# rednote-hilab/dots.ocr

Hardware: AMD Instinct MI355X
Metric: pages/sec, dots.ocr 1.7B bf16, A4@200dpi page batch (preprocess + ViT + prefill + 1024-token greedy decode + detokenise) (higher is better)
Workload: dtype bf16; 1 GPU; a4: 8 pages/GPU of 1654x2339 px -> 19824 patches, 5200 prompt tokens/page, max_new_tokens=1024, EOS disabled; pages_per_gpu=8, parallelism=dp1, decode_rows_in_flight=64

## Files before the change

### dots_ocr_amd/csrc/elementwise.hip

```cpp
#include "common.h"
#include "kernels.h"

namespace {

constexpr int MAX_CHUNKS = 8;

template <bool LAYERNORM, int NCH>
__global__ __launch_bounds__(256) void norm_kernel(const bf16_t* __restrict__ x, const bf16_t* __restrict__ w,
                                                   const bf16_t* __restrict__ b, bf16_t* __restrict__ y,
                                                   int64_t rows, int dim, float eps) {
    const int l = threadIdx.x & 63;
    const int64_t row = (int64_t)blockIdx.x * 4 + (threadIdx.x >> 6);
    if (row >= rows) return;
    const bf16_t* xr = x + row * dim;
    constexpr int NC = NCH > 0 ? NCH : MAX_CHUNKS;
    u32x4 v[NC];
    float s = 0.f, s2 = 0.f;
    if constexpr (NCH > 0) {
#pragma unroll
        for (int c = 0; c < NC; ++c) v[c] = *reinterpret_cast<const u32x4*>(xr + c * 512 + l * 8);
    }
#pragma unroll
    for (int c = 0; c < NC; ++c) {
        const int off = c * 512 + l * 8;
// ... 134 lines not shown
            const int item = it * 256 + tid;
            const int tok = item >> 4, c = item & 15;
            u32x4 v = {0, 0, 0, 0};
            if (tok < tl.n) v = *reinterpret_cast<const u32x4*>(qkv + (size_t)(tl.tok0 + tok) * ld + (Hq + Hkv + h) * 128 + c * 8);
            const int p = (tok & ~15) | (tok & 3) | (((tok >> 3) & 1) << 2) | (((tok >> 2) & 1) << 3);
            *reinterpret_cast<u32x4*>(&lds[p * 136 + c * 8]) = v;
        }
        __syncthreads();
#pragma unroll
        for (int it = 0; it < 4; ++it) {
            const int item = it * 256 + tid;
            const int d = item >> 3, pc = item & 7;
            u32x4 o;
#pragma unroll
            for (int e = 0; e < 4; ++e) {
                uint32_t a = lds[(pc * 8 + 2 * e) * 136 + d], b = lds[(pc * 8 + 2 * e + 1) * 136 + d];
                o[e] = a | (b << 16);
            }
            *reinterpret_cast<u32x4*>(vt + ((size_t)h * 128 + d) * Tpad + tl.pad0 + pc * 8) = o;
        }
    }
}

__global__ __launch_bounds__(256) void embed_gather_kernel(const int32_t* __restrict__ src, const bf16_t* __restrict__ embed,
                                                           const bf16_t* __restrict__ vision, bf16_t* __restrict__ x,
                                                           int64_t T, int dim) {
    const int l = threadIdx.x & 63;
    const int64_t t = (int64_t)blockIdx.x * 4 + (threadIdx.x >> 6);
    if (t >= T) return;
    const int sidx = src[t];
    const bf16_t* s = sidx >= 0 ? embed + (size_t)sidx * dim : vision + (size_t)(-sidx - 1) * dim;
    for (int off = l * 8; off < dim; off += 512)
        *reinterpret_cast<u32x4*>(x + t * dim + off) = *reinterpret_cast<const u32x4*>(s + off);
}

__global__ __launch_bounds__(256) void gather_rows_kernel(const bf16_t* __restrict__ x, const int32_t* __restrict__ rows,
                                                          const int32_t* __restrict__ dst, bf16_t* __restrict__ y, int n, int dim) {
    const int l = threadIdx.x & 63;
    const int r = blockIdx.x * 4 + (threadIdx.x >> 6);
    if (r >= n) return;
    const bf16_t* s = x + (size_t)rows[r] * dim;
    bf16_t* d = y + (size_t)(dst ? dst[r] : r) * dim;
    for (int off = l * 8; off < dim; off += 512) *reinterpret_cast<u32x4*>(d + off) = *reinterpret_cast<const u32x4*>(s + off);
}

}
// ... 23 lines not shown
hipError_t launch_patch_prep(hipStream_t s, const float* x, bf16_t* y, int64_t rows, int in_dim, int out_dim) {
    if (rows <= 0) return hipSuccess;
    if (in_dim % 4 != 0 || out_dim % 4 != 0 || out_dim < in_dim) return hipErrorInvalidValue;
    const int64_t n = rows * (out_dim / 4);
    hipLaunchKernelGGL(patch_prep_kernel, dim3((unsigned)((n + 255) / 256)), dim3(256), 0, s, x, y, rows, in_dim, out_dim);
    return hipGetLastError();
}

hipError_t launch_rope_table(hipStream_t s, const int32_t* pos, const float* inv_freq, float2* cs, int64_t T, int two_d) {
    if (T <= 0) return hipSuccess;
    hipLaunchKernelGGL(rope_table_kernel, dim3((unsigned)((T * 64 + 255) / 256)), dim3(256), 0, s, pos, inv_freq, cs, T, two_d);
    return hipGetLastError();
}

hipError_t launch_qkv_rope_split(hipStream_t s, const bf16_t* qkv, const float2* cs, const Tile64* tiles, int n_tiles,
                                 bf16_t* q, bf16_t* k, bf16_t* vt, int64_t T, int64_t Tpad, int Hq, int Hkv, bool v_only) {
    if (n_tiles <= 0) return hipSuccess;
    const int n_groups = (Hq + Hkv + ROPE_HPB - 1) / ROPE_HPB;
    if (v_only) hipLaunchKernelGGL(qkv_rope_split_kernel, dim3(n_tiles, Hkv), dim3(256), 0, s, qkv, cs, tiles, q, k, vt, T, Tpad, Hq, Hkv, n_groups);
    else hipLaunchKernelGGL(qkv_rope_split_kernel, dim3(n_tiles, n_groups + Hkv), dim3(256), 0, s, qkv, cs, tiles, q, k, vt, T, Tpad, Hq, Hkv, 0);
    return hipGetLastError();
}

hipError_t launch_embed_gather(hipStream_t s, const int32_t* src, const bf16_t* embed, const bf16_t* vision, bf16_t* x,
                               int64_t T, int dim) {
    if (T <= 0) return hipSuccess;
    hipLaunchKernelGGL(embed_gather_kernel, dim3((unsigned)((T + 3) / 4)), dim3(256), 0, s, src, embed, vision, x, T, dim);
    return hipGetLastError();
}

hipError_t launch_gather_rows(hipStream_t s, const bf16_t* x, const int32_t* rows, const int32_t* dst, bf16_t* y, int n, int dim) {
    if (n <= 0) return hipSuccess;
    hipLaunchKernelGGL(gather_rows_kernel, dim3((n + 3) / 4), dim3(256), 0, s, x, rows, dst, y, n, dim);
    return hipGetLastError();
}
```

### dots_ocr_amd/csrc/engine.hip

```cpp
#include <hip/hip_runtime.h>
#include <hip/hip_fp16.h>

#include <algorithm>
#include <cmath>
#include <cstdarg>
#include <cstddef>
#include <cstdio>
#include <cstdlib>
#include <cstring>
#include <string>
#include <unordered_map>
#include <vector>

#include "common.h"
#include "decode_layout.h"
#include "dots_ocr_hip.h"
#include "kernels.h"

namespace {

thread_local std::string g_create_error;

struct Tensor {
    bf16_t* p = nullptr;
// ... 86 lines not shown
    hipEvent_t ev_vis_ready = nullptr, ev_xs = nullptr;
    bf16_t* vis_pref = nullptr;
    int64_t vis_pref_rows = 0;
    bool pref_pending = false;
    bool pref_deferred = false;
    const float* pref_pix = nullptr;
    int64_t pref_patches = 0;
    std::vector<int64_t> pref_grid;
    hipStream_t vs = nullptr;
    hipStream_t s_vit_full = nullptr;
    hipEvent_t ev_tw0 = nullptr, ev_tw_sw = nullptr, ev_dec_end = nullptr;
    int tail_fixed = 0;
    int tail_now = 0;
    int tail_head_blocks = 0;
    uint64_t tw_seq = 0, dec_end_seq = 0, dec_end_at_tw = 0;
    std::vector<LLayer> ll;
    float *v_inv_freq = nullptr, *lm_inv_freq = nullptr;

    int64_t P = 0, Ppad = 0;
    bf16_t *v_xa = nullptr, *v_x = nullptr, *v_xn = nullptr, *v_qkv = nullptr, *v_q = nullptr, *v_k = nullptr, *v_vt = nullptr,
           *v_att = nullptr, *v_act = nullptr, *v_mh = nullptr, *vis = nullptr;
    float* v_pix = nullptr;
    float2* v_cs = nullptr;
    int32_t* v_pos = nullptr;
    Tile64* v_tiles = nullptr;
    QBlock* v_qblocks = nullptr;
    int64_t vis_rows = 0;
    std::vector<int32_t> h_pos;
    std::vector<Tile64> h_tiles;
    std::vector<QBlock> h_qblocks;

    int64_t TP = 0, TPpad = 0;
    bf16_t *p_x = nullptr, *p_xn = nullptr, *p_qkv = nullptr, *p_q = nullptr, *p_k = nullptr, *p_vt = nullptr, *p_att = nullptr, *p_act = nullptr;
    float2* p_cs = nullptr;
    int32_t *p_pos = nullptr, *p_src = nullptr, *p_last = nullptr;
    Tile64* p_tiles = nullptr;
    QBlock* p_qblocks = nullptr;
    std::vector<int32_t> hp_pos, hp_src, hp_last, hp_table;
    std::vector<Tile64> hp_tiles;
    std::vector<QBlock> hp_qblocks;

    int max_pages = 0;
    int n_pool_pages = 0;
    int kv_capped = 0;
    std::vector<int32_t> free_pages;
    std::vector<std::vector<int32_t>> slot_pages;
    bf16_t* pool = nullptr;
// ... 156 lines not shown
    return DOTS_OK;
}

int dense_on(DotsEngine* e, hipStream_t st, uint8_t* aq, float* as, const bf16_t* A, const bf16_t* W, const uint8_t* W8, const float* wscale,
             const bf16_t* bias, const bf16_t* R, void* C, int64_t M, int N, int K, int ldc, int epi) {
    if (!W8) {
        CK(launch_gemm(st, A, W, bias, R, C, M, N, K, K, ldc, epi, wscale));
        return DOTS_OK;
    }
    CK(launch_quant_act_fp8(st, A, aq, as, M, K, K));
    CK(launch_gemm_fp8(st, aq, as, W8, wscale, bias, R, C, M, N, K, ldc, epi));
    return DOTS_OK;
}
int dense(DotsEngine* e, const bf16_t* A, const bf16_t* W, const uint8_t* W8, const float* wscale, const bf16_t* bias, const bf16_t* R, void* C,
          int64_t M, int N, int K, int ldc, int epi) {
    return dense_on(e, e->stream, e->act_q, e->act_s, A, W, W8, wscale, bias, R, C, M, N, K, ldc, epi);
}
int vdense(DotsEngine* e, const bf16_t* A, const bf16_t* W, const uint8_t* W8, const float* wscale, const bf16_t* bias, const bf16_t* R, void* C,
           int64_t M, int N, int K, int ldc, int epi) {
    return dense_on(e, e->vs, e->act_q_v, e->act_s_v, A, W, W8, wscale, bias, R, C, M, N, K, ldc, epi);
}

int qkv_rope_on(DotsEngine* e, hipStream_t st, uint8_t* aq, float* as, const bf16_t* A, const bf16_t* W, const uint8_t* W8, const float* wscale, const bf16_t* bias,
                bf16_t* qkv, const float2* cs, const Tile64* tiles, int n_tiles, bf16_t* q, bf16_t* k, bf16_t* vt, int64_t T, int64_t Tpad, int K, int Hq, int Hkv) {
    const int N = (Hq + 2 * Hkv) * 128;
    if (!W8 && !wscale) {
        const hipError_t r = launch_gemm_qk_rope(st, A, W, bias, qkv, T, N, K, K, N, cs, q, k, Hq, Hkv);
        if (r == hipSuccess) {
            CK(launch_qkv_rope_split(st, qkv, cs, tiles, n_tiles, q, k, vt, T, Tpad, Hq, Hkv, true));
            return DOTS_OK;
        }
        if (r != hipErrorNotSupported) CK(r);
    }
    RET(dense_on(e, st, aq, as, A, W, W8, wscale, bias, nullptr, qkv, T, N, K, N, EPI_NONE));
    CK(launch_qkv_rope_split(st, qkv, cs, tiles, n_tiles, q, k, vt, T, Tpad, Hq, Hkv));
    return DOTS_OK;
}

int decode_copy(DotsEngine* e, const bf16_t* W, void** out, int64_t rows, int K, int rot_rows) {
    const size_t elems = (size_t)((rows + 15) / 16 * 16) * K;
    if (e->cfg.fp8_weights) {
        uint8_t* d = nullptr;
        CK(e->alloc(&d, elems));
        CK(launch_pack_frag_fp8(e->stream, W, d, rows, K, rot_rows));
        *out = d;
    } else {
        bf16_t* d = nullptr;
        CK(e->alloc(&d, elems));
        if (rot_rows) CK(launch_pack_frag_qkv(e->stream, W, d, e->cfg.num_heads, e->cfg.num_kv_heads, K));
        else CK(launch_pack_frag(e->stream, W, d, rows, K));
        *out = d;
    }
    return DOTS_OK;
}

int finalize_weights(DotsEngine* e) {
    const DotsConfig& c = e->cfg;
    hipStream_t s = e->stream;
    const int E = c.v_embed_dim, Iv = c.v_intermediate;
// ... 138 lines not shown
    if (c.fp8_weights) {
        const size_t v_max = (size_t)e->P * std::max(E, c.v_intermediate);
        const size_t p_max = (size_t)c.max_prefill_tokens * std::max(H, std::max(Nq, c.intermediate_size));
        CK(e->alloc(&e->act_q, p_max));
        CK(e->alloc(&e->act_s, (size_t)c.max_prefill_tokens));
        CK(e->alloc(&e->act_q_v, v_max));
        CK(e->alloc(&e->act_s_v, (size_t)e->P));
    }
    CK(e->alloc(&e->v_xa, (size_t)e->P * kpad));
    CK(e->alloc(&e->v_x, (size_t)e->P * E));
    CK(e->alloc(&e->v_xn, (size_t)e->P * E));
    CK(e->alloc(&e->v_qkv, (size_t)e->P * 3 * E));
    CK(e->alloc(&e->v_q, (size_t)e->P * E));
    CK(e->alloc(&e->v_k, (size_t)(e->P + 64) * E));
    CK(e->alloc(&e->v_vt, (size_t)e->Ppad * E));
    CK(e->alloc(&e->v_att, (size_t)e->P * E));
    CK(e->alloc(&e->v_act, (size_t)e->P * c.v_intermediate));
    CK(e->alloc(&e->v_mh, (size_t)(e->P / 4 + 1) * Mg));
    CK(e->alloc(&e->vis, (size_t)(e->P / 4 + 1) * H));
    CK(e->alloc(&e->vis_pref, (size_t)(e->P / 4 + 1) * H));
    CK(e->alloc(&e->v_cs, (size_t)e->P * 64));
    CK(e->alloc(&e->v_pos, (size_t)e->P * 2));
    CK(e->alloc(&e->v_tiles, (size_t)(e->P / 64 + 256)));
    CK(e->alloc(&e->v_qblocks, (size_t)(e->P / 128 + 256) * c.v_heads));

    e->TP = c.max_prefill_tokens;
    e->TPpad = e->TP + 64 * c.max_batch;
    CK(e->alloc(&e->p_x, (size_t)e->TP * H));
    CK(e->alloc(&e->p_xn, (size_t)e->TP * H));
    CK(e->alloc(&e->p_qkv, (size_t)e->TP * (Nq + 2 * Nkv)));
    CK(e->alloc(&e->p_q, (size_t)e->TP * Nq));
    CK(e->alloc(&e->p_k, (size_t)(e->TP + 64) * Nkv));
    CK(e->alloc(&e->p_vt, (size_t)e->TPpad * Nkv));
    CK(e->alloc(&e->p_att, (size_t)e->TP * Nq));
    CK(e->alloc(&e->p_act, (size_t)e->TP * c.intermediate_size));
    CK(e->alloc(&e->p_cs, (size_t)e->TP * 64));
    CK(e->alloc(&e->p_pos, (size_t)e->TP));
    CK(e->alloc(&e->p_src, (size_t)e->TP));
    CK(e->alloc(&e->p_last, (size_t)DOTS_MAX_BATCH));
    CK(e->alloc(&e->p_tiles, (size_t)(e->TP / 64 + c.max_batch + 1)));
    CK(e->alloc(&e->p_qblocks, (size_t)(e->TP / 128 + c.max_batch + 1) * c.num_heads));

    e->max_pages = (c.max_seq_len + 63) / 64;
    const int64_t pool_tokens = c.kv_pool_tokens > 0 ? c.kv_pool_tokens : (int64_t)c.max_batch * e->max_pages * 64;
    e->n_pool_pages = (int)((pool_tokens + 63) / 64);
    e->kv8 = c.kv_cache_dtype == 1;
// ... 151 lines not shown
                    for (int mh = 0; mh < m; ++mh)
                        for (int mw = 0; mw < m; ++mw) {
                            e->h_pos[off * 2] = (int32_t)(gh * m + mh);
                            e->h_pos[off * 2 + 1] = (int32_t)(gw * m + mw);
                            ++off;
                        }
            lens.push_back((int)(h * w));
            attn_flops += 4.0 * (double)(h * w) * (double)(h * w) * E;
        }
    }
    if (off != N) return e->fail(DOTS_E_INVALID, "grid_thw covers %lld patches, total_patches is %lld", (long long)off, (long long)N);
    if (lens.size() > 256) return e->fail(DOTS_E_CAPACITY, "more than 256 images per call");
    int64_t Tpad = 0;
    build_worklists(lens, Hh, e->h_tiles, e->h_qblocks, &Tpad);
    CK(hipMemcpyAsync(e->v_pos, e->h_pos.data(), e->h_pos.size() * 4, hipMemcpyHostToDevice, s));
    CK(hipMemcpyAsync(e->v_tiles, e->h_tiles.data(), e->h_tiles.size() * sizeof(Tile64), hipMemcpyHostToDevice, s));
    CK(hipMemcpyAsync(e->v_qblocks, e->h_qblocks.data(), e->h_qblocks.size() * sizeof(QBlock), hipMemcpyHostToDevice, s));

    CK(hipEventRecord(e->ev[0], s));
    CK(launch_patch_prep(s, pix_dev, e->v_xa, N, e->patch_k, e->patch_kpad));
    CK(launch_gemm(s, e->v_xa, e->patch_w, e->patch_b, nullptr, e->v_xn, N, E, e->patch_kpad, e->patch_kpad, E, EPI_NONE));
    CK(launch_rmsnorm(s, e->v_xn, e->patch_norm, e->v_x, N, E, c.v_rms_eps));
    CK(launch_rope_table(s, e->v_pos, e->v_inv_freq, e->v_cs, N, 1));
    const float scale = 1.0f / sqrtf(128.0f);
    e->attn_pairs = 0;
    const XcdPlan xcd_plan = make_xcd_plan(e->h_qblocks.data(), (int)e->h_qblocks.size());
    hipStream_t const s_first = s;
    const bool prefetched = e->s_vit && s == e->s_vit && e->s_vit_full;
    const int switch_at = prefetched ? c.v_layers - std::max(0, std::min(e->tail_now, c.v_layers - 1)) : -1;
    if (prefetched) CK(hipEventRecord(e->ev_tw0, s));
    for (int i = 0; i < c.v_layers; ++i) {
        const VLayer& L = e->vl[i];
        if (i == switch_at) {
            CK(hipEventRecord(e->ev_tw_sw, s));
            e->tail_head_blocks = i;
            RET(chain_streams(e, s, e->s_vit_full));
            e->vs = s = e->s_vit_full;
        }
        CK(launch_rmsnorm(s, e->v_x, L.norm1, e->v_xn, N, E, c.v_rms_eps));
        RET(qkv_rope_on(e, s, e->act_q_v, e->act_s_v, e->v_xn, L.qkv_w, L.qkv_8, L.qkv_s, L.qkv_b, e->v_qkv, e->v_cs, e->v_tiles, (int)e->h_tiles.size(), e->v_q, e->v_k, e->v_vt,
                        N, Tpad, E, Hh, Hh));
        CK(attn_event(e, 2 * i));
        CK(launch_flash_attn(s, e->v_q, e->v_k, e->v_vt, e->v_att, e->v_qblocks, (int)e->h_qblocks.size(), N, Tpad, Hh, Hh, 0, scale, &xcd_plan));
        CK(attn_event(e, 2 * i + 1));
        e->attn_pairs = i + 1;
        RET(vdense(e, e->v_att, L.proj_w, L.proj_8, L.proj_s, L.proj_b, e->v_x, e->v_x, N, E, E, E, EPI_RESIDUAL));
        CK(launch_rmsnorm(s, e->v_x, L.norm2, e->v_xn, N, E, c.v_rms_eps));
        RET(vdense(e, e->v_xn, L.w13, L.w13_8, L.w13_s, L.b13, nullptr, e->v_act, N, 2 * c.v_intermediate, E, c.v_intermediate, EPI_SWIGLU));
        RET(vdense(e, e->v_act, L.w2, L.w2_8, L.w2_s, L.b2, e->v_x, e->v_x, N, E, c.v_intermediate, E, EPI_RESIDUAL));
        if (e->dbg_hidden && (size_t)(i + 1) * N * E <= e->dbg_cap) {
            CK(hipMemcpyAsync(e->dbg_hidden + (size_t)i * N * E, e->v_x, (size_t)N * E * 2, hipMemcpyDeviceToDevice, s));
            e->dbg_vit_rows = N;
        }
    }
    if (prefetched && switch_at == c.v_layers) {
        CK(hipEventRecord(e->ev_tw_sw, s));
        e->tail_head_blocks = c.v_layers;
    }
    const bf16_t* xin = e->v_x;
    if (c.v_post_norm) {
        CK(launch_rmsnorm(s, e->v_x, e->v_post_norm, e->v_xn, N, E, c.v_rms_eps));
        xin = e->v_xn;
    }
    CK(launch_layernorm(s, xin, e->m_ln_w, e->m_ln_b, e->v_att, N, E, c.v_ln_eps));
// ... 1660 lines not shown
    if (!e || !x || !w || !qkv_ws || !q || !k || !vt || !cu || n_seq < 1 || !pos_host) return DOTS_E_INVALID;
    CK(hipSetDevice(e->device));
    std::vector<Tile64> tiles;
    std::vector<QBlock> qb;
    Tile64* dt = nullptr;
    QBlock* dq = nullptr;
    int64_t Tpad = 0;
    RET(upload_lists(e, cu, n_seq, Hq, tiles, qb, &dt, &dq, &Tpad));
    const int64_t T = cu[n_seq];
    const int N = (Hq + 2 * Hkv) * 128;
    int32_t* dpos = nullptr;
    float2* cs = nullptr;
    float* freq = nullptr;
    const int nf = rope2d ? 32 : 64;
    std::vector<float> f(nf);
    for (int i = 0; i < nf; ++i) f[i] = 1.0f / powf(theta, (float)(2 * i) / (rope2d ? 64.0f : 128.0f));
    CK(e->alloc(&dpos, (size_t)T * (rope2d ? 2 : 1)));
    CK(e->alloc(&cs, (size_t)T * 64));
    CK(e->alloc(&freq, (size_t)nf));
    CK(hipMemcpyAsync(dpos, pos_host, (size_t)T * (rope2d ? 2 : 1) * 4, hipMemcpyHostToDevice, e->stream));
    CK(hipMemcpyAsync(freq, f.data(), nf * 4, hipMemcpyHostToDevice, e->stream));
    CK(launch_rope_table(e->stream, dpos, freq, cs, T, rope2d));
    hipError_t r;
    if (fused) {
        r = launch_gemm_qk_rope(e->stream, (const bf16_t*)x, (const bf16_t*)w, (const bf16_t*)bias, (bf16_t*)qkv_ws, T, N, K, K, N, cs, (bf16_t*)q, (bf16_t*)k, Hq, Hkv);
        if (r == hipSuccess) r = launch_qkv_rope_split(e->stream, (const bf16_t*)qkv_ws, cs, dt, (int)tiles.size(), (bf16_t*)q, (bf16_t*)k, (bf16_t*)vt, T, Tpad, Hq, Hkv, true);
    } else {
        r = launch_gemm(e->stream, (const bf16_t*)x, (const bf16_t*)w, (const bf16_t*)bias, nullptr, qkv_ws, T, N, K, K, N, EPI_NONE);
        if (r == hipSuccess) r = launch_qkv_rope_split(e->stream, (const bf16_t*)qkv_ws, cs, dt, (int)tiles.size(), (bf16_t*)q, (bf16_t*)k, (bf16_t*)vt, T, Tpad, Hq, Hkv);
    }
    hipStreamSynchronize(e->stream);
    e->release(dt); e->release(dq); e->release(dpos); e->release(cs); e->release(freq);
    if (r == hipErrorNotSupported) { (void)hipGetLastError(); return e->fail(DOTS_E_INVALID, "no fused qkv + rope kernel for this shape / GEMM plan"); }
    CK(r);
    return DOTS_OK;
}


namespace {
int op_dec_qkv(DotsEngine* e, const void* h, const void* ln_w, const void* wqkv, const void* bias, const int32_t* ctx_len_dev,
               const int32_t* block_table_dev, int max_pages, void* pool_layer, void* q_out, int B, int H, int Hq, int Hkv, float eps,
               float rope_theta, int fp8, const float* kv_scales) {
    if (!e || !h || !ln_w || !wqkv || !ctx_len_dev || !block_table_dev || !pool_layer || !q_out) return e ? e->fail(DOTS_E_INVALID, "null argument") : DOTS_E_INVALID;
    CK(hipSetDevice(e->device));
    Scratch sc(e);
    void* wd = nullptr;
    float *freq = nullptr, *wscale = nullptr;
    CK(sc.get(&freq, 64));
    float f[64];
    for (int i = 0; i < 64; ++i) f[i] = 1.0f / powf(rope_theta, (float)(2 * i) / 128.0f);
    CK(hipMemcpyAsync(freq, f, sizeof(f), hipMemcpyHostToDevice, e->stream));
    RET(op_weight(e, sc, (const bf16_t*)wqkv, (int64_t)(Hq + 2 * Hkv) * 128, H, Hq, Hkv, true, fp8, &wd, &wscale));
    bf16_t* xn = nullptr;
    CK(sc.get(&xn, (size_t)DOTS_MAX_BATCH * H));
    CK(launch_dec_qkv(e->stream, (const bf16_t*)h, (const bf16_t*)ln_w, wd, wscale, (const bf16_t*)bias, freq, ctx_len_dev, block_table_dev, max_pages,
// ... 386 lines not shown
```

### dots_ocr_amd/csrc/gemm.hip

```cpp
#include <cstdlib>
#include <utility>

#include "common.h"
#include "kernels.h"

namespace {

constexpr int BM = 128, BN = 128, BK = 64;
constexpr int TILE_BYTES = 128 * 128;
#ifndef GEMM_GROUP_M
#define GEMM_GROUP_M 8
#endif
constexpr int GROUP_M = GEMM_GROUP_M;

DEVI float gelu_erf(float x) { return 0.5f * x * (1.0f + erff(x * 0.70710678118654752440f)); }
#ifdef GEMM_EXACT_SILU
DEVI float silu(float x) { return x / (1.0f + __expf(-x)); }
#else
DEVI float silu(float x) {
    const float d = 1.0f + __expf(fminf(-x, 80.f));
    const float r = __builtin_amdgcn_rcpf(d);
    const float q = x * r;
    return __builtin_fmaf(__builtin_fmaf(-q, d, x), r, q);
}
// ... 631 lines not shown
            float u[8] = {a[it][2][0], a[it][2][1], a[it][2][2], a[it][2][3], a[it][3][0], a[it][3][1], a[it][3][2], a[it][3][3]};
            if (has_cols) {
#pragma unroll
                for (int e = 0; e < 8; ++e) { o[e] = o[e] * cc.sc0[e] + cc.bi0[e]; u[e] = u[e] * cc.sc1[e] + cc.bi1[e]; }
            }
            uint32_t pk[4];
#pragma unroll
            for (int e = 0; e < 4; ++e) {
                const uint32_t ow = pack_bf2(o[2 * e], o[2 * e + 1]), uw = pack_bf2(u[2 * e], u[2 * e + 1]);
                const float x0 = lo_bf(ow), x1 = hi_bf(ow), y0 = lo_bf(uw), y1 = hi_bf(uw);
                const f32x4 t4 = tb[qb & 1][it][e];
                const float f0 = lo_half ? x0 : y0, g0 = lo_half ? t4[0] : t4[1], m0 = lo_half ? y0 : x0, n0_ = lo_half ? t4[1] : t4[0];
                const float p0 = m0 * n0_, p1 = y1 * t4[3];
                const float r0 = __builtin_fmaf(f0, g0, lo_half ? -p0 : p0), r1 = __builtin_fmaf(x1, t4[2], lo_half ? -p1 : p1);
                pk[e] = pack_bf2(r0, r1);
            }
            if (FULL || m < M) *reinterpret_cast<u32x4*>(dst + (size_t)m * 128 + gcol) = u32x4{pk[0], pk[1], pk[2], pk[3]};
        }
        __builtin_amdgcn_sched_barrier(0);
    }
#undef W4_PUT
}

template <int... I, class F> DEVI void gemm_static_for_impl(std::integer_sequence<int, I...>, F&& f) { (f(std::integral_constant<int, I>{}), ...); }
template <int N, class F> DEVI void gemm_static_for(F&& f) { gemm_static_for_impl(std::make_integer_sequence<int, N>{}, f); }

template <int EPI>
DEVI void gemm_bf16_w4_body(
    const bf16_t* __restrict__ A, const bf16_t* __restrict__ W, const bf16_t* __restrict__ bias,
    const float* __restrict__ colscale, const bf16_t* R, void* Cout, int M, int N, int K, int lda, int ldc, int m_tiles, int n_tiles, int group_m, const QkRope& rope) {
    extern __shared__ __attribute__((aligned(16))) char smem2[];
    (void)rope;

    const int tid = threadIdx.x;
    const int l = tid & 63;
    const int w = __builtin_amdgcn_readfirstlane(tid >> 6);
    const int hi = l >> 5, l31 = l & 31;

    int bid = xcd_remap(blockIdx.x, m_tiles * n_tiles);
    const int per_group = group_m * n_tiles;
    const int g = bid / per_group;
    const int first_m = g * group_m;
    const int gsz = min(m_tiles - first_m, group_m);
    const int in_grp = bid - g * per_group;
    const int tm = first_m + in_grp % gsz;
    const int tn = in_grp / gsz;
// ... 1 lines not shown

    const int prow = 8 * w + (l >> 3);
    const int chunk = ((l & 7) ^ ((4 * w + (l >> 4)) & 7)) << 4;
    const int w_src = prow * (K * 2) + chunk;
    int x_src[8];
#pragma unroll
    for (int i = 0; i < 8; ++i) x_src[i] = (min(m0 + prow + 32 * i, M - 1) - m0) * (lda * 2) + chunk;
    const __amdgpu_buffer_rsrc_t rw = __builtin_amdgcn_make_buffer_rsrc((void*)(W + (size_t)n0 * K), 0, 0x7ffffff0, 0x00020000);
    const __amdgpu_buffer_rsrc_t rx = __builtin_amdgcn_make_buffer_rsrc((void*)(A + (size_t)m0 * lda), 0, 0x7ffffff0, 0x00020000);
    const int w_step = 32 * K * 2;
    auto dma_w = [&](int t, int slot, int i) {
        __builtin_amdgcn_raw_ptr_buffer_load_lds(rw, (__attribute__((address_space(3))) void*)(smem2 + slot * W4_UNIT + (w + 4 * i) * 1024), 16, w_src,
                                                 t * 128 + i * w_step, 0, 0);
    };
    auto dma_x = [&](int t, int slot, int i) {
        __builtin_amdgcn_raw_ptr_buffer_load_lds(rx, (__attribute__((address_space(3))) void*)(smem2 + slot * W4_UNIT + (w + 4 * i) * 1024), 16, x_src[i],
                                                 t * 128, 0, 0);
    };

    const int wn = w >> 1, wm = w & 1;
    const int rsw = (l31 >> 1) & 7;
    const int lane_sw = ((hi ^ (rsw & 1)) << 4) | ((rsw >> 1) << 5);
    const int lds0 = (int)(uintptr_t)(__attribute__((address_space(3))) char*)smem2;
    const int a_lane = lds0 + (wn * 128 + l31) * 128 + lane_sw;
    const int b_lane = lds0 + (wm * 128 + l31) * 128 + lane_sw;
    auto frag = [&](int base, int ks, int f) {
        return *reinterpret_cast<const __attribute__((address_space(3))) bf16x8*>((uintptr_t)(uint32_t)((base ^ (ks << 5)) + f * 4096));
    };

#ifdef W4_PROF
    const unsigned long long pt0 = __builtin_amdgcn_s_memtime(), pw0 = wall_clock64();
#endif
    W4Cols cols;
    if constexpr (EPI == EPI_QKROPE) w4_load_cols_rope(cols, bias, colscale, n0 + wn * 128, l);
    else if constexpr (EPI != EPI_F32) w4_load_cols<EPI == EPI_SWIGLU>(cols, bias, colscale, n0 + wn * 128, l);

    f32x16 acc[4][4];
#pragma unroll
    for (int i = 0; i < 4; ++i)
#pragma unroll
        for (int j = 0; j < 4; ++j)
#pragma unroll
            for (int r = 0; r < 16; ++r) acc[i][j][r] = 0.f;

    const int nt = K / BK;
#ifdef W4_STAGGER
    if (blockIdx.x < 256) {
        const int naps = ((blockIdx.x >> 3) & 7) * nt * W4_STAGGER / 8;
        for (int i = 0; i < naps; ++i) __builtin_amdgcn_s_sleep(8);
    }
#endif
#pragma unroll
    for (int u = 0; u < 4; ++u)
#pragma unroll
        for (int i = 0; i < 8; ++i) {
            if (u & 1) dma_x(u >> 1, u, i);
            else dma_w(u >> 1, u, i);
        }
    asm volatile("s_waitcnt vmcnt(16)" ::: "memory");
    __builtin_amdgcn_s_barrier();
    bf16x8 fa[2][4], fb[2][4];
#pragma unroll
    for (int f = 0; f < 4; ++f) { fa[0][f] = frag(a_lane, 0, f); fb[0][f] = frag(b_lane + W4_UNIT, 0, f); }
#ifdef W4_PROF
    const unsigned long long pt1 = __builtin_amdgcn_s_memtime(), pw1 = wall_clock64();
#endif

    auto tile_body = [&](auto mode_c, int t, int u0) {
        constexpr int MODE = decltype(mode_c)::value;
        const int s1 = u0 + 1 >= W4_RING ? u0 + 1 - W4_RING : u0 + 1, s2 = u0 + 2 >= W4_RING ? u0 + 2 - W4_RING : u0 + 2;
        const int s3 = u0 + 3 >= W4_RING ? u0 + 3 - W4_RING : u0 + 3, s4 = u0 + 4 >= W4_RING ? u0 + 4 - W4_RING : u0 + 4;
        const int aw = a_lane + u0 * W4_UNIT, ax = b_lane + s1 * W4_UNIT;
        const int awn = a_lane + s2 * W4_UNIT, axn = b_lane + s3 * W4_UNIT;
        gemm_static_for<64>([&acc, &fa, &fb, &frag, &dma_w, &dma_x, aw, ax, awn, axn, t, u0, s4](auto gc) {
            constexpr int gp = decltype(gc)::value;
            (void)acc; (void)t; (void)u0; (void)s4; (void)dma_w; (void)dma_x;
            constexpr int ks = gp >> 4, idx = gp & 15, fn = idx >> 2, fm = idx & 3, cur = ks & 1;
            if constexpr (gp == 48 && MODE < 2) {
                if constexpr (MODE == 0) asm volatile("s_waitcnt vmcnt(8) lgkmcnt(0)" ::: "memory");
                else asm volatile("s_waitcnt vmcnt(0) lgkmcnt(0)" ::: "memory");
                __builtin_amdgcn_s_barrier();
            }
            if constexpr (idx < 8 && (ks < 3 || MODE < 2)) {
                constexpr int f = idx & 3;
                if constexpr (ks < 3) {
                    if constexpr (idx < 4) fa[cur ^ 1][f] = frag(aw, ks + 1, f);
                    else fb[cur ^ 1][f] = frag(ax, ks + 1, f);
                } else {
                    if constexpr (idx < 4) fa[cur ^ 1][f] = frag(awn, 0, f);
                    else fb[cur ^ 1][f] = frag(axn, 0, f);
                }
            }
#ifndef W4_NO_DMA
            if constexpr (MODE == 0) {
                if constexpr (gp == 8 || gp == 11 || gp == 14 || gp == 24 || gp == 27 || gp == 30 || gp == 40 || gp == 43) {
                    constexpr int i = gp < 16 ? (gp - 8) / 3 : gp < 32 ? 3 + (gp - 24) / 3 : 6 + (gp - 40) / 3;
// ... 19 lines not shown
#endif
    __syncthreads();
#ifdef W4_NO_STORE
#pragma unroll
    for (int i = 0; i < 4; ++i)
#pragma unroll
        for (int j = 0; j < 4; ++j) asm volatile("" ::"a"(acc[i][j]));
    return;
#endif
#ifdef W4_OLD_EPILOGUE
    if constexpr (EPI == EPI_F32 || EPI == EPI_SWIGLU) {
        gemm_epilogue<EPI, 4, 4>(acc, bias, colscale, R, Cout, M, ldc, n0 + wn * 128, m0 + wm * 128, l31, hi);
    } else {
        gemm_epilogue_lds<EPI, 4>(acc, bias, colscale, R, reinterpret_cast<bf16_t*>(Cout), M, ldc, n0 + wn * 128, m0 + wm * 128, l, smem2 + w * 16384);
    }
#else
    if constexpr (EPI == EPI_QKROPE) {
        const int head = (n0 + wn * 128) >> 7;
        const bool full = m0 + wm * 128 + 128 <= M, has_cols = bias != nullptr || colscale != nullptr;
        if (head < rope.n_rope_heads) {
            bf16_t* dst = head < rope.Hq ? rope.q + (size_t)head * rope.T * 128 : rope.k + (size_t)(head - rope.Hq) * rope.T * 128;
            if (full) w4_epilogue_qkrope<true>(acc, cols, has_cols, rope.cs, dst, M, m0 + wm * 128, l, smem2 + w * 32768);
            else w4_epilogue_qkrope<false>(acc, cols, has_cols, rope.cs, dst, M, m0 + wm * 128, l, smem2 + w * 32768);
        } else if (full) {
            w4_epilogue_lds<EPI_NONE, true>(acc, cols, has_cols, R, reinterpret_cast<bf16_t*>(Cout), M, ldc, n0 + wn * 128, m0 + wm * 128, l, smem2 + w * 32768);
        } else {
            w4_epilogue_lds<EPI_NONE, false>(acc, cols, has_cols, R, reinterpret_cast<bf16_t*>(Cout), M, ldc, n0 + wn * 128, m0 + wm * 128, l, smem2 + w * 32768);
        }
    } else if constexpr (EPI == EPI_F32) {
        gemm_epilogue<EPI, 4, 4>(acc, bias, colscale, R, Cout, M, ldc, n0 + wn * 128, m0 + wm * 128, l31, hi);
    } else if (m0 + wm * 128 + 128 <= M) {
        w4_epilogue_lds<EPI, true>(acc, cols, bias != nullptr || colscale != nullptr, R, reinterpret_cast<bf16_t*>(Cout), M, ldc, n0 + wn * 128, m0 + wm * 128, l, smem2 + w * 32768);
    } else {
        w4_epilogue_lds<EPI, false>(acc, cols, bias != nullptr || colscale != nullptr, R, reinterpret_cast<bf16_t*>(Cout), M, ldc, n0 + wn * 128, m0 + wm * 128, l, smem2 + w * 32768);
    }
#endif
#ifdef W4_PROF
    const unsigned long long pt2b = __builtin_amdgcn_s_memtime();
    asm volatile("s_waitcnt vmcnt(0)" ::: "memory");
    const unsigned long long pt3 = __builtin_amdgcn_s_memtime(), pw3 = wall_clock64();
    if ((blockIdx.x == 1000 || blockIdx.x == 2001 || blockIdx.x == 3002) && tid == 0)
        printf("W4_PROF epi %d N %d K %d blk %d: prologue %llu cyc / %.2f us, main loop %llu cyc / %.2f us (%.0f cyc per K tile), epilogue + drain %llu cyc / %.2f us; issue %llu drain %llu\n", EPI, N, K,
               (int)blockIdx.x, pt1 - pt0, (pw1 - pw0) * 0.01, pt2 - pt1, (pw2 - pw1) * 0.01, (double)(pt2 - pt1) / nt, pt3 - pt2, (pw3 - pw2) * 0.01, pt2b - pt2, pt3 - pt2b);
#endif
}

// ... 196 lines not shown
            case EPI_GELU: return launch_256<EPI_GELU>(s, A, W, bias, colscale, R, C, (int)M, N, K, lda, ldc);
            case EPI_F32: return launch_256<EPI_F32>(s, A, W, bias, colscale, R, C, (int)M, N, K, lda, ldc);
            default: return hipErrorInvalidValue;
        }
    }
    const int m_tiles = (int)((M + BM - 1) / BM), n_tiles = N / BN;
    dim3 grid(m_tiles * n_tiles), block(256);
#define LAUNCH(E)                                                                                       \
    hipLaunchKernelGGL(gemm_bf16_kernel<E>, grid, block, 0, s, A, W, bias, colscale, R, C, (int)M, N, K, lda, ldc, \
                       m_tiles, n_tiles)
    switch (epi) {
        case EPI_NONE: LAUNCH(EPI_NONE); break;
        case EPI_RESIDUAL: LAUNCH(EPI_RESIDUAL); break;
        case EPI_SWIGLU: LAUNCH(EPI_SWIGLU); break;
        case EPI_GELU: LAUNCH(EPI_GELU); break;
        case EPI_F32: LAUNCH(EPI_F32); break;
        default: return hipErrorInvalidValue;
    }
#undef LAUNCH
    return hipGetLastError();
}

hipError_t launch_gemm_qk_rope(hipStream_t s, const bf16_t* A, const bf16_t* W, const bf16_t* bias, bf16_t* qkv, int64_t M, int N, int K, int lda, int ldc,
                               const float2* cs, bf16_t* q, bf16_t* k, int Hq, int Hkv) {
    static const bool off = getenv("DOTS_OCR_QK_FUSE") && atoi(getenv("DOTS_OCR_QK_FUSE")) == 0;
    static const bool lockstep = getenv("DOTS_OCR_GEMM_LOCKSTEP") != nullptr, force_small = getenv("DOTS_OCR_GEMM_128") != nullptr;
    if (off || lockstep || force_small || gemm_get_plan() != 1 || N != (Hq + 2 * Hkv) * 128 || N % BN2 != 0 || K % BK != 0 || K / BK < 3 || lda % 8 != 0 || ldc % 8 != 0 ||
        !cs || !q || !k || M > 0x7fffffff)
        return hipErrorNotSupported;
    if (M <= 0) return hipSuccess;
    static uint32_t configured = 0;
    int dev = 0;
    hipError_t e = hipGetDevice(&dev);
    if (e != hipSuccess) return e;
    const uint32_t bit = 1u << (dev & 31);
    if (!(__atomic_load_n(&configured, __ATOMIC_ACQUIRE) & bit)) {
        e = hipFuncSetAttribute(reinterpret_cast<const void*>(&gemm_bf16_w4_qkrope_kernel), hipFuncAttributeMaxDynamicSharedMemorySize, W4_RING * W4_UNIT);
        if (e != hipSuccess) return e;
        __atomic_fetch_or(&configured, bit, __ATOMIC_RELEASE);
    }
    const int m_tiles = (int)((M + BM2 - 1) / BM2), n_tiles = N / BN2;
    const QkRope rope{cs, q, k, (long long)M, Hq, Hq + Hkv};
    hipLaunchKernelGGL(gemm_bf16_w4_qkrope_kernel, dim3(m_tiles * n_tiles), dim3(256), W4_RING * W4_UNIT, s, A, W, bias, (const float*)nullptr, (void*)qkv, (int)M, N, K,
                       lda, ldc, m_tiles, n_tiles, raster_group_m(K * 2), rope);
    return hipGetLastError();
}

bool gemm_fp8_supports(int N, int K) { return N % BN2 == 0 && K % 64 == 0; }

template <int E>
static hipError_t launch_fp8_t(hipStream_t s, const uint8_t* Aq, const float* rowscale, const uint8_t* Wq, const float* colscale, const bf16_t* bias,
                               const bf16_t* R, void* C, int M, int N, int K, int ldc) {
    static uint32_t configured = 0;
    int dev = 0;
    hipError_t e = hipGetDevice(&dev);
    if (e != hipSuccess) return e;
    const uint32_t bit = 1u << (dev & 31);
    if (!(__atomic_load_n(&configured, __ATOMIC_ACQUIRE) & bit)) {
        e = hipFuncSetAttribute(reinterpret_cast<const void*>(&gemm_fp8_256pp_kernel<E>), hipFuncAttributeMaxDynamicSharedMemorySize, PP_STAGES * SUB_STAGE);
        if (e != hipSuccess) return e;
        __atomic_fetch_or(&configured, bit, __ATOMIC_RELEASE);
    }
    const int m_tiles = (M + BM2 - 1) / BM2, n_tiles = N / BN2;
    hipLaunchKernelGGL(gemm_fp8_256pp_kernel<E>, dim3(m_tiles * n_tiles), dim3(512), PP_STAGES * SUB_STAGE, s, Aq, rowscale, Wq, colscale, bias, R, C, M, N, K,
                       ldc, m_tiles, n_tiles, raster_group_m(K));
// ... 16 lines not shown
```

### dots_ocr_amd/csrc/kernels.h

```cpp
#pragma once
#include <hip/hip_runtime.h>
#include <stdint.h>

typedef uint16_t bf16_t;

#define DOTS_MAX_BATCH 64

enum { EPI_NONE = 0, EPI_RESIDUAL = 1, EPI_SWIGLU = 2, EPI_GELU = 3, EPI_F32 = 4, EPI_QKROPE = 5  };

hipError_t launch_gemm(hipStream_t s, const bf16_t* A, const bf16_t* W, const bf16_t* bias, const bf16_t* R,
                       void* C, int64_t M, int N, int K, int lda, int ldc, int epi, const float* colscale = nullptr);
int gemm_get_plan();
void gemm_set_plan(int plan);

hipError_t launch_rmsnorm(hipStream_t s, const bf16_t* x, const bf16_t* w, bf16_t* y, int64_t rows, int dim, float eps);
hipError_t launch_layernorm(hipStream_t s, const bf16_t* x, const bf16_t* w, const bf16_t* b, bf16_t* y,
                            int64_t rows, int dim, float eps);
hipError_t launch_patch_prep(hipStream_t s, const float* x, bf16_t* y, int64_t rows, int in_dim, int out_dim);
hipError_t launch_rope_table(hipStream_t s, const int32_t* pos, const float* inv_freq, float2* cs, int64_t T, int two_d);
struct Tile64 { int32_t tok0, n, pad0, seq, page, _pad; };
hipError_t launch_qkv_rope_split(hipStream_t s, const bf16_t* qkv, const float2* cs, const Tile64* tiles, int n_tiles,
                                 bf16_t* q, bf16_t* k, bf16_t* vt, int64_t T, int64_t Tpad, int Hq, int Hkv, bool v_only = false);
struct QkRope { const float2* cs; bf16_t* q; bf16_t* k; long long T; int Hq; int n_rope_heads; };
hipError_t launch_gemm_qk_rope(hipStream_t s, const bf16_t* A, const bf16_t* W, const bf16_t* bias, bf16_t* qkv, int64_t M, int N, int K, int lda, int ldc,
                               const float2* cs, bf16_t* q, bf16_t* k, int Hq, int Hkv);
hipError_t launch_embed_gather(hipStream_t s, const int32_t* src, const bf16_t* embed, const bf16_t* vision, bf16_t* x,
                               int64_t T, int dim);
hipError_t launch_gather_rows(hipStream_t s, const bf16_t* x, const int32_t* rows, const int32_t* dst, bf16_t* y, int n, int dim);

struct QBlock { int32_t q0, n, tok0, pad0, head, _pad; };
int flash_rows_per_block();
struct XcdPlan { int32_t base[8], cnt[8]; };
XcdPlan make_xcd_plan(const QBlock* blocks_host, int n_blocks);
hipError_t launch_flash_attn(hipStream_t s, const bf16_t* q, const bf16_t* k, const bf16_t* vt, bf16_t* out,
                             const QBlock* blocks, int n_blocks, int64_t T, int64_t Tpad, int Hq, int Hkv,
                             int causal, float scale, const XcdPlan* plan = nullptr);

hipError_t launch_kv_to_pages(hipStream_t s, const bf16_t* k, const bf16_t* qkv, const Tile64* tiles, int n_tiles,
                              const int32_t* block_table, int max_pages, void* pool_layer, int64_t T, int Hq, int Hkv,
                              const float* kv_scales = nullptr);
hipError_t launch_dec_embed(hipStream_t s, const int32_t* tokens, const bf16_t* embed, bf16_t* h, int B, int dim);
hipError_t launch_dec_qkv(hipStream_t s, const bf16_t* h, const bf16_t* ln_w, const void* Wd, const float* wscale, const bf16_t* bias,
                          const float* inv_freq, const int32_t* ctx_len, const int32_t* block_table, int max_pages,
                          void* pool_layer, bf16_t* q_out, int B, int H, int Hq, int Hkv, float eps, int part_cus = 0, bf16_t* xn = nullptr,
                          const float* pend = nullptr, const float* pend_scale = nullptr, const float* kv_scales = nullptr);
hipError_t launch_dec_proj(hipStream_t s, const bf16_t* X, const void* Wd, const float* wscale, bf16_t* h, int B, int N, int K, int part_cus = 0,
                           float* part = nullptr, bool* pending = nullptr);
hipError_t launch_dec_gateup(hipStream_t s, const bf16_t* h, const bf16_t* ln_w, const void* W13d, const float* wscale, bf16_t* act,
// ... 121 lines not shown
```

Baseline: 6.155 pages/s.

## Write transposed V directly from fused QKV GEMM epilogue in ViT

Adds a V-transpose epilogue to the fused QKV+RoPE GEMM. For V heads the warp swaps its A/B operand roles so the accumulator comes out already transposed, and it writes the result straight into the padded vt layout through a per-16-token position map. This removes the separate qkv_rope_split pass over V (a read of qkv plus a transposing write) on every ViT layer. A small prepare kernel builds the map and zeroes tile padding once per forward. The path only applies when all sequence lengths are multiples of 16, the weights are not fp8 and the head count is even, and it adds complexity to the GEMM inner loop.

```diff
diff --git a/dots_ocr_amd/csrc/elementwise.hip b/dots_ocr_amd/csrc/elementwise.hip
--- a/dots_ocr_amd/csrc/elementwise.hip
+++ b/dots_ocr_amd/csrc/elementwise.hip
@@ -180,6 +180,15 @@
     }
 }
 
+__global__ __launch_bounds__(256) void vt_prepare_kernel(const Tile64* __restrict__ tiles, int32_t* __restrict__ vmap, bf16_t* __restrict__ vt, int64_t Tpad) {
+    const Tile64 tl = tiles[blockIdx.x];
+    const int tid = threadIdx.x;
+    if (blockIdx.y == 0 && tid * 16 < tl.n) vmap[(tl.tok0 >> 4) + tid] = tl.pad0 + tid * 16;
+    if (tl.n == 64) return;
+    bf16_t* row = vt + (size_t)(blockIdx.y * 256 + tid) * Tpad + tl.pad0;
+    for (int p = tl.n; p < 64; p += 8) *reinterpret_cast<u32x4*>(row + p) = u32x4{0, 0, 0, 0};
+}
+
 __global__ __launch_bounds__(256) void embed_gather_kernel(const int32_t* __restrict__ src, const bf16_t* __restrict__ embed,
                                                            const bf16_t* __restrict__ vision, bf16_t* __restrict__ x,
                                                            int64_t T, int dim) {
@@ -249,6 +258,13 @@
     return hipGetLastError();
 }
 
+hipError_t launch_vt_prepare(hipStream_t s, const Tile64* tiles, int n_tiles, int32_t* vmap, bf16_t* vt, int64_t Tpad, int Hkv) {
+    if (n_tiles <= 0) return hipSuccess;
+    if (Hkv < 1 || Hkv % 2 != 0) return hipErrorInvalidValue;
+    hipLaunchKernelGGL(vt_prepare_kernel, dim3(n_tiles, Hkv / 2), dim3(256), 0, s, tiles, vmap, vt, Tpad);
+    return hipGetLastError();
+}
+
 hipError_t launch_embed_gather(hipStream_t s, const int32_t* src, const bf16_t* embed, const bf16_t* vision, bf16_t* x,
                                int64_t T, int dim) {
     if (T <= 0) return hipSuccess;
diff --git a/dots_ocr_amd/csrc/engine.hip b/dots_ocr_amd/csrc/engine.hip
--- a/dots_ocr_amd/csrc/engine.hip
+++ b/dots_ocr_amd/csrc/engine.hip
@@ -132,7 +132,7 @@
            *v_att = nullptr, *v_act = nullptr, *v_mh = nullptr, *vis = nullptr;
     float* v_pix = nullptr;
     float2* v_cs = nullptr;
-    int32_t* v_pos = nullptr;
+    int32_t *v_pos = nullptr, *v_vmap = nullptr;
     Tile64* v_tiles = nullptr;
     QBlock* v_qblocks = nullptr;
     int64_t vis_rows = 0;
@@ -335,12 +335,13 @@
 }
 
 int qkv_rope_on(DotsEngine* e, hipStream_t st, uint8_t* aq, float* as, const bf16_t* A, const bf16_t* W, const uint8_t* W8, const float* wscale, const bf16_t* bias,
-                bf16_t* qkv, const float2* cs, const Tile64* tiles, int n_tiles, bf16_t* q, bf16_t* k, bf16_t* vt, int64_t T, int64_t Tpad, int K, int Hq, int Hkv) {
+                bf16_t* qkv, const float2* cs, const Tile64* tiles, int n_tiles, bf16_t* q, bf16_t* k, bf16_t* vt, int64_t T, int64_t Tpad, int K, int Hq, int Hkv,
+                const int32_t* vmap = nullptr) {
     const int N = (Hq + 2 * Hkv) * 128;
     if (!W8 && !wscale) {
-        const hipError_t r = launch_gemm_qk_rope(st, A, W, bias, qkv, T, N, K, K, N, cs, q, k, Hq, Hkv);
+        const hipError_t r = launch_gemm_qk_rope(st, A, W, bias, qkv, T, N, K, K, N, cs, q, k, Hq, Hkv, vmap, vt, Tpad);
         if (r == hipSuccess) {
-            CK(launch_qkv_rope_split(st, qkv, cs, tiles, n_tiles, q, k, vt, T, Tpad, Hq, Hkv, true));
+            if (!vmap) CK(launch_qkv_rope_split(st, qkv, cs, tiles, n_tiles, q, k, vt, T, Tpad, Hq, Hkv, true));
             return DOTS_OK;
         }
         if (r != hipErrorNotSupported) CK(r);
@@ -348,6 +349,11 @@
     RET(dense_on(e, st, aq, as, A, W, W8, wscale, bias, nullptr, qkv, T, N, K, N, EPI_NONE));
     CK(launch_qkv_rope_split(st, qkv, cs, tiles, n_tiles, q, k, vt, T, Tpad, Hq, Hkv));
     return DOTS_OK;
+}
+bool vt_epilogue_fits(const int* lens, size_t n) {
+    for (size_t i = 0; i < n; ++i)
+        if (lens[i] % 16 != 0) return false;
+    return true;
 }
 
 int decode_copy(DotsEngine* e, const bf16_t* W, void** out, int64_t rows, int K, int rot_rows) {
@@ -532,6 +538,7 @@
     CK(e->alloc(&e->v_cs, (size_t)e->P * 64));
     CK(e->alloc(&e->v_pos, (size_t)e->P * 2));
     CK(e->alloc(&e->v_tiles, (size_t)(e->P / 64 + 256)));
+    CK(e->alloc(&e->v_vmap, (size_t)(e->P / 16 + 16)));
     CK(e->alloc(&e->v_qblocks, (size_t)(e->P / 128 + 256) * c.v_heads));
 
     e->TP = c.max_prefill_tokens;
@@ -729,6 +736,11 @@
     CK(launch_gemm(s, e->v_xa, e->patch_w, e->patch_b, nullptr, e->v_xn, N, E, e->patch_kpad, e->patch_kpad, E, EPI_NONE));
     CK(launch_rmsnorm(s, e->v_xn, e->patch_norm, e->v_x, N, E, c.v_rms_eps));
     CK(launch_rope_table(s, e->v_pos, e->v_inv_freq, e->v_cs, N, 1));
+    const int32_t* vmap = nullptr;
+    if (!c.fp8_weights && Hh % 2 == 0 && vt_epilogue_fits(lens.data(), lens.size())) {
+        CK(launch_vt_prepare(s, e->v_tiles, (int)e->h_tiles.size(), e->v_vmap, e->v_vt, Tpad, Hh));
+        vmap = e->v_vmap;
+    }
     const float scale = 1.0f / sqrtf(128.0f);
     e->attn_pairs = 0;
     const XcdPlan xcd_plan = make_xcd_plan(e->h_qblocks.data(), (int)e->h_qblocks.size());
@@ -746,7 +758,7 @@
         }
         CK(launch_rmsnorm(s, e->v_x, L.norm1, e->v_xn, N, E, c.v_rms_eps));
         RET(qkv_rope_on(e, s, e->act_q_v, e->act_s_v, e->v_xn, L.qkv_w, L.qkv_8, L.qkv_s, L.qkv_b, e->v_qkv, e->v_cs, e->v_tiles, (int)e->h_tiles.size(), e->v_q, e->v_k, e->v_vt,
-                        N, Tpad, E, Hh, Hh));
+                        N, Tpad, E, Hh, Hh, vmap));
         CK(attn_event(e, 2 * i));
         CK(launch_flash_attn(s, e->v_q, e->v_k, e->v_vt, e->v_att, e->v_qblocks, (int)e->h_qblocks.size(), N, Tpad, Hh, Hh, 0, scale, &xcd_plan));
         CK(attn_event(e, 2 * i + 1));
@@ -2453,15 +2465,26 @@
     CK(hipMemcpyAsync(freq, f.data(), nf * 4, hipMemcpyHostToDevice, e->stream));
     CK(launch_rope_table(e->stream, dpos, freq, cs, T, rope2d));
     hipError_t r;
+    int32_t* vmap = nullptr;
+    if (fused == 2 && Hkv % 2 == 0) {
+        std::vector<int> lens(n_seq);
+        for (int i = 0; i < n_seq; ++i) lens[i] = cu[i + 1] - cu[i];
+        if (vt_epilogue_fits(lens.data(), lens.size())) CK(e->alloc(&vmap, (size_t)(T / 16 + 1)));
+    }
     if (fused) {
-        r = launch_gemm_qk_rope(e->stream, (const bf16_t*)x, (const bf16_t*)w, (const bf16_t*)bias, (bf16_t*)qkv_ws, T, N, K, K, N, cs, (bf16_t*)q, (bf16_t*)k, Hq, Hkv);
-        if (r == hipSuccess) r = launch_qkv_rope_split(e->stream, (const bf16_t*)qkv_ws, cs, dt, (int)tiles.size(), (bf16_t*)q, (bf16_t*)k, (bf16_t*)vt, T, Tpad, Hq, Hkv, true);
+        r = vmap ? launch_vt_prepare(e->stream, dt, (int)tiles.size(), vmap, (bf16_t*)vt, Tpad, Hkv) : hipSuccess;
+        if (r == hipSuccess)
+            r = launch_gemm_qk_rope(e->stream, (const bf16_t*)x, (const bf16_t*)w, (const bf16_t*)bias, (bf16_t*)qkv_ws, T, N, K, K, N, cs, (bf16_t*)q, (bf16_t*)k, Hq, Hkv,
+                                    vmap, (bf16_t*)vt, Tpad);
+        if (r == hipSuccess && !vmap)
+            r = launch_qkv_rope_split(e->stream, (const bf16_t*)qkv_ws, cs, dt, (int)tiles.size(), (bf16_t*)q, (bf16_t*)k, (bf16_t*)vt, T, Tpad, Hq, Hkv, true);
     } else {
         r = launch_gemm(e->stream, (const bf16_t*)x, (const bf16_t*)w, (const bf16_t*)bias, nullptr, qkv_ws, T, N, K, K, N, EPI_NONE);
         if (r == hipSuccess) r = launch_qkv_rope_split(e->stream, (const bf16_t*)qkv_ws, cs, dt, (int)tiles.size(), (bf16_t*)q, (bf16_t*)k, (bf16_t*)vt, T, Tpad, Hq, Hkv);
     }
     hipStreamSynchronize(e->stream);
     e->release(dt); e->release(dq); e->release(dpos); e->release(cs); e->release(freq);
+    if (vmap) e->release(vmap);
     if (r == hipErrorNotSupported) { (void)hipGetLastError(); return e->fail(DOTS_E_INVALID, "no fused qkv + rope kernel for this shape / GEMM plan"); }
     CK(r);
     return DOTS_OK;
diff --git a/dots_ocr_amd/csrc/gemm.hip b/dots_ocr_amd/csrc/gemm.hip
--- a/dots_ocr_amd/csrc/gemm.hip
+++ b/dots_ocr_amd/csrc/gemm.hip
@@ -677,6 +677,58 @@
 #undef W4_PUT
 }
 
+DEVI void w4_epilogue_vt(const f32x16 (&acc)[4][4], const W4Cols& cc, bool has_bias, const int32_t* __restrict__ vmap, bf16_t* __restrict__ vth, long long Tpad,
+                         int M, int mw0, int l, char* stage2) {
+    const int hi = l >> 5, l31 = l & 31, rrow = l >> 4, run = l & 15;
+    const int grp = (mw0 >> 4) + (run >> 1);
+    const bool vok = grp * 16 < M;
+    const int vpos = vmap[min(grp, (M >> 4) - 1)] + (run & 1) * 8;
+    auto swz = [](int row) { return ((row & 15) << 1) ^ (row & 1) ^ ((row & 2) << 2); };
+    const int wslot = swz(l31);
+    char* const wrow = stage2 + l31 * 512;
+#define W4_PUT(FM, IMG)                                                                                                   \
+    _Pragma("unroll") for (int fn = 0; fn < 4; ++fn) _Pragma("unroll") for (int rq = 0; rq < 4; ++rq) {                     \
+        const f32x4 v = {acc[fn][FM][4 * rq], acc[fn][FM][4 * rq + 1], acc[fn][FM][4 * rq + 2], acc[fn][FM][4 * rq + 3]};   \
+        *reinterpret_cast<f32x4*>(wrow + (IMG) * 16384 + (((fn * 8 + rq * 2 + hi) ^ wslot) << 4)) = v;                      \
+    }
+    const int s0 = 8 * (run >> 2) + 4 * ((run >> 1) & 1) + (run & 1);
+    bf16_t* const out = vth + (size_t)rrow * Tpad + vpos;
+    W4_PUT(0, 0)
+#pragma unroll
+    for (int b = 0; b < 4; ++b) {
+        if (b + 1 < 4) {
+            if (b == 0) { W4_PUT(1, 1) } else if (b == 1) { W4_PUT(2, 0) } else { W4_PUT(3, 1) }
+        }
+        __builtin_amdgcn_sched_barrier(0);
+        const char* img = stage2 + (b & 1) * 16384;
+        f32x4 v[8][2];
+#pragma unroll
+        for (int it = 0; it < 8; ++it) {
+            const int row = it * 4 + rrow;
+            const int sw = swz(row);
+            const char* rp = img + row * 512;
+            v[it][0] = *reinterpret_cast<const f32x4*>(rp + ((s0 ^ sw) << 4));
+            v[it][1] = *reinterpret_cast<const f32x4*>(rp + (((s0 + 2) ^ sw) << 4));
+        }
+        __builtin_amdgcn_sched_barrier(0);
+#pragma unroll
+        for (int it = 0; it < 8; ++it) {
+            const float bi = b == 0 ? cc.sc0[it] : b == 1 ? cc.bi0[it] : b == 2 ? cc.sc1[it] : cc.bi1[it];
+            float o[8] = {v[it][0][0], v[it][0][1], v[it][0][2], v[it][0][3], v[it][1][0], v[it][1][1], v[it][1][2], v[it][1][3]};
+            if (has_bias) {
+#pragma unroll
+                for (int e = 0; e < 8; ++e) o[e] += bi;
+            }
+            if (vok) {
+                const u32x4 pk = {pack_bf2(o[0], o[1]), pack_bf2(o[2], o[3]), pack_bf2(o[4], o[5]), pack_bf2(o[6], o[7])};
+                *reinterpret_cast<u32x4*>(out + (size_t)(b * 32 + it * 4) * Tpad) = pk;
+            }
+        }
+        __builtin_amdgcn_sched_barrier(0);
+    }
+#undef W4_PUT
+}
+
 template <int... I, class F> DEVI void gemm_static_for_impl(std::integer_sequence<int, I...>, F&& f) { (f(std::integral_constant<int, I>{}), ...); }
 template <int N, class F> DEVI void gemm_static_for(F&& f) { gemm_static_for_impl(std::make_integer_sequence<int, N>{}, f); }
 
@@ -724,8 +776,12 @@
     const int rsw = (l31 >> 1) & 7;
     const int lane_sw = ((hi ^ (rsw & 1)) << 4) | ((rsw >> 1) << 5);
     const int lds0 = (int)(uintptr_t)(__attribute__((address_space(3))) char*)smem2;
-    const int a_lane = lds0 + (wn * 128 + l31) * 128 + lane_sw;
-    const int b_lane = lds0 + (wm * 128 + l31) * 128 + lane_sw;
+    bool vswap = false;
+    if constexpr (EPI == EPI_QKROPE) vswap = rope.vt != nullptr && ((n0 + wn * 128) >> 7) >= rope.n_rope_heads;
+    int wa = wn, wb = wm;
+    if constexpr (EPI == EPI_QKROPE) { wa = vswap ? wm : wn; wb = vswap ? wn : wm; }
+    const int a_lane = lds0 + (wa * 128 + l31) * 128 + lane_sw;
+    const int b_lane = lds0 + (wb * 128 + l31) * 128 + lane_sw;
     auto frag = [&](int base, int ks, int f) {
         return *reinterpret_cast<const __attribute__((address_space(3))) bf16x8*>((uintptr_t)(uint32_t)((base ^ (ks << 5)) + f * 4096));
     };
@@ -734,7 +790,20 @@
     const unsigned long long pt0 = __builtin_amdgcn_s_memtime(), pw0 = wall_clock64();
 #endif
     W4Cols cols;
-    if constexpr (EPI == EPI_QKROPE) w4_load_cols_rope(cols, bias, colscale, n0 + wn * 128, l);
+    if constexpr (EPI == EPI_QKROPE) {
+        if (vswap) {
+#pragma unroll
+            for (int it = 0; it < 8; ++it) {
+                const bf16_t* bp = bias + n0 + wn * 128 + 4 * it + (l >> 4);
+                cols.sc0[it] = bias ? __uint_as_float((uint32_t)bp[0] << 16) : 0.f;
+                cols.bi0[it] = bias ? __uint_as_float((uint32_t)bp[32] << 16) : 0.f;
+                cols.sc1[it] = bias ? __uint_as_float((uint32_t)bp[64] << 16) : 0.f;
+                cols.bi1[it] = bias ? __uint_as_float((uint32_t)bp[96] << 16) : 0.f;
+            }
+        } else {
+            w4_load_cols_rope(cols, bias, colscale, n0 + wn * 128, l);
+        }
+    }
     else if constexpr (EPI != EPI_F32) w4_load_cols<EPI == EPI_SWIGLU>(cols, bias, colscale, n0 + wn * 128, l);
 
     f32x16 acc[4][4];
@@ -763,7 +832,10 @@
     __builtin_amdgcn_s_barrier();
     bf16x8 fa[2][4], fb[2][4];
 #pragma unroll
-    for (int f = 0; f < 4; ++f) { fa[0][f] = frag(a_lane, 0, f); fb[0][f] = frag(b_lane + W4_UNIT, 0, f); }
+    for (int f = 0; f < 4; ++f) {
+        if constexpr (EPI == EPI_QKROPE) { fa[0][f] = frag(a_lane + (vswap ? W4_UNIT : 0), 0, f); fb[0][f] = frag(b_lane + (vswap ? 0 : W4_UNIT), 0, f); }
+        else { fa[0][f] = frag(a_lane, 0, f); fb[0][f] = frag(b_lane + W4_UNIT, 0, f); }
+    }
 #ifdef W4_PROF
     const unsigned long long pt1 = __builtin_amdgcn_s_memtime(), pw1 = wall_clock64();
 #endif
@@ -772,8 +844,10 @@
         constexpr int MODE = decltype(mode_c)::value;
         const int s1 = u0 + 1 >= W4_RING ? u0 + 1 - W4_RING : u0 + 1, s2 = u0 + 2 >= W4_RING ? u0 + 2 - W4_RING : u0 + 2;
         const int s3 = u0 + 3 >= W4_RING ? u0 + 3 - W4_RING : u0 + 3, s4 = u0 + 4 >= W4_RING ? u0 + 4 - W4_RING : u0 + 4;
-        const int aw = a_lane + u0 * W4_UNIT, ax = b_lane + s1 * W4_UNIT;
-        const int awn = a_lane + s2 * W4_UNIT, axn = b_lane + s3 * W4_UNIT;
+        int ua = u0, ub = s1, uan = s2, ubn = s3;
+        if constexpr (EPI == EPI_QKROPE) { ua = vswap ? s1 : u0; ub = vswap ? u0 : s1; uan = vswap ? s3 : s2; ubn = vswap ? s2 : s3; }
+        const int aw = a_lane + ua * W4_UNIT, ax = b_lane + ub * W4_UNIT;
+        const int awn = a_lane + uan * W4_UNIT, axn = b_lane + ubn * W4_UNIT;
         gemm_static_for<64>([&acc, &fa, &fb, &frag, &dma_w, &dma_x, aw, ax, awn, axn, t, u0, s4](auto gc) {
             constexpr int gp = decltype(gc)::value;
             (void)acc; (void)t; (void)u0; (void)s4; (void)dma_w; (void)dma_x;
@@ -839,6 +913,9 @@
             bf16_t* dst = head < rope.Hq ? rope.q + (size_t)head * rope.T * 128 : rope.k + (size_t)(head - rope.Hq) * rope.T * 128;
             if (full) w4_epilogue_qkrope<true>(acc, cols, has_cols, rope.cs, dst, M, m0 + wm * 128, l, smem2 + w * 32768);
             else w4_epilogue_qkrope<false>(acc, cols, has_cols, rope.cs, dst, M, m0 + wm * 128, l, smem2 + w * 32768);
+        } else if (vswap) {
+            w4_epilogue_vt(acc, cols, bias != nullptr, rope.vmap, rope.vt + (size_t)(head - rope.n_rope_heads) * 128 * rope.Tpad, rope.Tpad, M, m0 + wm * 128, l,
+                           smem2 + w * 32768);
         } else if (full) {
             w4_epilogue_lds<EPI_NONE, true>(acc, cols, has_cols, R, reinterpret_cast<bf16_t*>(Cout), M, ldc, n0 + wn * 128, m0 + wm * 128, l, smem2 + w * 32768);
         } else {
@@ -1081,13 +1158,14 @@
 }
 
 hipError_t launch_gemm_qk_rope(hipStream_t s, const bf16_t* A, const bf16_t* W, const bf16_t* bias, bf16_t* qkv, int64_t M, int N, int K, int lda, int ldc,
-                               const float2* cs, bf16_t* q, bf16_t* k, int Hq, int Hkv) {
+                               const float2* cs, bf16_t* q, bf16_t* k, int Hq, int Hkv, const int32_t* vmap, bf16_t* vt, int64_t Tpad) {
     static const bool off = getenv("DOTS_OCR_QK_FUSE") && atoi(getenv("DOTS_OCR_QK_FUSE")) == 0;
     static const bool lockstep = getenv("DOTS_OCR_GEMM_LOCKSTEP") != nullptr, force_small = getenv("DOTS_OCR_GEMM_128") != nullptr;
     if (off || lockstep || force_small || gemm_get_plan() != 1 || N != (Hq + 2 * Hkv) * 128 || N % BN2 != 0 || K % BK != 0 || K / BK < 3 || lda % 8 != 0 || ldc % 8 != 0 ||
         !cs || !q || !k || M > 0x7fffffff)
         return hipErrorNotSupported;
     if (M <= 0) return hipSuccess;
+    if (vmap && (!vt || M % 16 != 0 || Tpad % 64 != 0)) return hipErrorInvalidValue;
     static uint32_t configured = 0;
     int dev = 0;
     hipError_t e = hipGetDevice(&dev);
@@ -1099,7 +1177,7 @@
         __atomic_fetch_or(&configured, bit, __ATOMIC_RELEASE);
     }
     const int m_tiles = (int)((M + BM2 - 1) / BM2), n_tiles = N / BN2;
-    const QkRope rope{cs, q, k, (long long)M, Hq, Hq + Hkv};
+    const QkRope rope{cs, q, k, (long long)M, Hq, Hq + Hkv, vmap, vmap ? vt : nullptr, (long long)Tpad};
     hipLaunchKernelGGL(gemm_bf16_w4_qkrope_kernel, dim3(m_tiles * n_tiles), dim3(256), W4_RING * W4_UNIT, s, A, W, bias, (const float*)nullptr, (void*)qkv, (int)M, N, K,
                        lda, ldc, m_tiles, n_tiles, raster_group_m(K * 2), rope);
     return hipGetLastError();
diff --git a/dots_ocr_amd/csrc/kernels.h b/dots_ocr_amd/csrc/kernels.h
--- a/dots_ocr_amd/csrc/kernels.h
+++ b/dots_ocr_amd/csrc/kernels.h
@@ -21,9 +21,10 @@
 struct Tile64 { int32_t tok0, n, pad0, seq, page, _pad; };
 hipError_t launch_qkv_rope_split(hipStream_t s, const bf16_t* qkv, const float2* cs, const Tile64* tiles, int n_tiles,
                                  bf16_t* q, bf16_t* k, bf16_t* vt, int64_t T, int64_t Tpad, int Hq, int Hkv, bool v_only = false);
-struct QkRope { const float2* cs; bf16_t* q; bf16_t* k; long long T; int Hq; int n_rope_heads; };
+struct QkRope { const float2* cs; bf16_t* q; bf16_t* k; long long T; int Hq; int n_rope_heads; const int32_t* vmap; bf16_t* vt; long long Tpad; };
 hipError_t launch_gemm_qk_rope(hipStream_t s, const bf16_t* A, const bf16_t* W, const bf16_t* bias, bf16_t* qkv, int64_t M, int N, int K, int lda, int ldc,
-                               const float2* cs, bf16_t* q, bf16_t* k, int Hq, int Hkv);
+                               const float2* cs, bf16_t* q, bf16_t* k, int Hq, int Hkv, const int32_t* vmap = nullptr, bf16_t* vt = nullptr, int64_t Tpad = 0);
+hipError_t launch_vt_prepare(hipStream_t s, const Tile64* tiles, int n_tiles, int32_t* vmap, bf16_t* vt, int64_t Tpad, int Hkv);
 hipError_t launch_embed_gather(hipStream_t s, const int32_t* src, const bf16_t* embed, const bf16_t* vision, bf16_t* x,
                                int64_t T, int dim);
 hipError_t launch_gather_rows(hipStream_t s, const bf16_t* x, const int32_t* rows, const int32_t* dst, bf16_t* y, int n, int dim);
```

Result: no change. 6.160 pages/s, median of 2 (+0.1%).
